# ShijieZhou-UCLA/feature-3dgs

Measured on NVIDIA H100. Metric: views/sec fwd+bwd @1M Gaussians/1080p/feat_dim=128, higher is better.
Workload: dtype f32

## Files before the change

### feature-3dgs_b200/csrc/composite_common.cuh

```cuda
#pragma once
#include <initializer_list>

#include "kernels.h"

namespace f3dgs {

constexpr int kBlocksPerTile = 8;
constexpr int kProducerWarp = 0;
constexpr int kAlphaWarp0 = 4;
constexpr int kAlphaWarps = kBlocksPerTile;
constexpr int kFeatWarp0 = kAlphaWarp0 + kAlphaWarps;
constexpr int kRegsProducer = 40;
constexpr int kStageEntries = 32;
constexpr int kStages = 6;
constexpr int kWSlots = 2;
constexpr int kDoneSlots = 8;

template <int CH, typename TF = float>
struct alignas(128) Stage {
    TF feat[CH > 0 ? kStageEntries : 1][CH > 0 ? CH : 4];
    float4 rec0[kStageEntries];
    float4 rec1[kStageEntries];
    float4 rec2[kStageEntries];
    uint32_t listpos[kStageEntries];
    uint32_t gid[kStageEntries];
    uint32_t n;
    uint32_t last;
    uint32_t first;
    int32_t work;
    uint32_t done_slot;
};

struct alignas(128) WSlot {
    float w[kStageEntries][32];
    uint32_t pm[kStageEntries];
    uint32_t km[2];
    uint32_t last;
    uint32_t first;
    int32_t work;
};
static_assert(sizeof(WSlot) == 4352, "weight slot layout changed");

constexpr int kPrefetch = 4;
struct alignas(16) RecQueue {
    float4 q[kPrefetch][3][32];
    uint32_t id[kPrefetch][32];
};

template <int CH, typename TF = float, int WB = kBlocksPerTile, int WJ = kWSlots>
struct alignas(128) RingV2 {
    using Feat = TF;
    static constexpr int kWB = WB, kWJ = WJ;
    Stage<CH, TF> stage[kStages];
    WSlot ws[WB][WJ];
    uint64_t full[kStages];
    uint64_t empty[kStages];
    uint64_t listed[kStages];
    uint64_t wfull[WB][WJ];
    uint64_t wempty[WB][WJ];
    uint32_t done_mask[kDoneSlots];
    RecQueue rq;
};

using RingSlim = RingV2<0, float, 1, 1>;

static_assert(sizeof(RecQueue) == 6656, "record queue layout changed");
static_assert(sizeof(RingV2<0>) == 88320 && sizeof(RingSlim) == 22784, "ring layout changed");
static_assert(sizeof(RingV2<32>) == 112896 && sizeof(RingV2<64>) == 137472 && sizeof(RingV2<128>) == 186624,
              "ring layout changed");
static_assert(sizeof(RingV2<32, __half>) == 100608 && sizeof(RingV2<64, __half>) == 112896 &&
                  sizeof(RingV2<128, __half>) == 137472,
              "ring layout changed");

__device__ __forceinline__ int block_x0(int tile_x, int b) { return tile_x * 16 + (b & 1) * 8; }
__device__ __forceinline__ int block_y0(int tile_y, int b) { return tile_y * 16 + (b >> 1) * 4; }
__device__ __forceinline__ int slot_px(int p) { return ((p >> 2) & 3) * 2 + (p & 1); }
__device__ __forceinline__ int slot_py(int p) { return (p >> 4) * 2 + ((p >> 1) & 1); }

template <int NQ>
__device__ __forceinline__ float& tile_px(float2 (&t)[NQ][2][4], int qi, int i, int c) {
    return (i & 1) ? t[qi][i >> 1][c].y : t[qi][i >> 1][c].x;
}
template <int NQ>
__device__ __forceinline__ float& tile_run_px(float2 (&t)[NQ][2][4], int y, int half, int k, int c) {
    return tile_px(t, ((y >> 1) * 4 + half * 2 + (k >> 1)) % NQ, (y & 1) * 2 + (k & 1), c);
}
template <int NQ>
__device__ __forceinline__ float4 tile_run(float2 (&t)[NQ][2][4], int y, int half, int c) {
    return make_float4(tile_run_px(t, y, half, 0, c), tile_run_px(t, y, half, 1, c), tile_run_px(t, y, half, 2, c),
                       tile_run_px(t, y, half, 3, c));
}
template <int NQ>
__device__ __forceinline__ void set_tile_run(float2 (&t)[NQ][2][4], int y, int half, int c, float4 v) {
    tile_run_px(t, y, half, 0, c) = v.x;
    tile_run_px(t, y, half, 1, c) = v.y;
    tile_run_px(t, y, half, 2, c) = v.z;
    tile_run_px(t, y, half, 3, c) = v.w;
}

template <int G, int NQ, int NY = 4, typename T, class Row, class Run, class Px>
__device__ __forceinline__ void for_tile_pixels(T* plane, int bx0, int by0, int W, int H, int grp, bool rows, bool runs,
                                                Row row, Run run, Px px) {
    static_assert(NQ * G * 2 == NY * 4, "a register tile of NQ quads per lane group covers NY rows of 8 pixels");
    if (G == 1 && rows && bx0 + 8 <= W) {
#pragma unroll
        for (int y = 0; y < NY; y++) {
            const int yy = by0 + y;
            if (yy >= H) continue;
            row(plane + (size_t)yy * W + bx0, y);
        }
    } else if (G == 1 && runs) {
#pragma unroll
        for (int y = 0; y < NY; y++) {
            const int yy = by0 + y;
            if (yy >= H) continue;
#pragma unroll
            for (int half = 0; half < 2; half++) {
                const int xx = bx0 + half * 4;
                if (xx >= W) continue;
                run(plane + (size_t)yy * W + xx, y, half);
            }
        }
    } else {
#pragma unroll
        for (int qi = 0; qi < NQ; qi++) {
            const int q = qi * G + grp;
#pragma unroll
            for (int i = 0; i < 4; i++) {
                const int xx = bx0 + (q & 3) * 2 + (i & 1), yy = by0 + (q >> 2) * 2 + (i >> 1);
                if (xx < W && yy < H) px(plane + (size_t)yy * W + xx, qi, i);
            }
        }
    }
}

__device__ __forceinline__ float4 to_float4(float4 v) { return v; }
__device__ __forceinline__ float4 to_float4(uint2 v) {
    const float2 a = __half22float2(*reinterpret_cast<const __half2*>(&v.x));
    const float2 b = __half22float2(*reinterpret_cast<const __half2*>(&v.y));
    return make_float4(a.x, a.y, b.x, b.y);
}

struct InstanceLists {
    float* w;
    uint2* meta;
    uint32_t* cnt;
};

__device__ __forceinline__ size_t list_begin(uint32_t begin, uint32_t end, int b) {
    return kBlocksPerTile * (size_t)begin + (size_t)b * (end - begin);
}

struct ListLayout {
    size_t w, meta, cnt, bytes;
    ListLayout(size_t R, size_t tiles) {
        size_t o = 0;
        w = o;     o = align_up(o + kBlocksPerTile * R * 32 * sizeof(float));
        meta = o;  o = align_up(o + kBlocksPerTile * R * sizeof(uint2));
        cnt = o;   o = align_up(o + kBlocksPerTile * tiles * sizeof(uint32_t));
        bytes = o;
    }
};

constexpr int kCounterFwd = 0, kCounterBwdGeom = 16, kCounterFeatureBwd = 48;

template <typename TG>
cudaError_t launch_feature_bwd(const ViewParams& vp, const uint2* ranges, const InstanceLists& lists,
                               const TG* dL_dfeat_pix, float dL_dfeat_pix_scale, float* dL_dfeature, int* counters,
                               cudaStream_t s);

struct SplatAlpha {
    float dx, dy, G, alpha;
};
__device__ __forceinline__ SplatAlpha splat_alpha(const float4 r0, const float4 r1, float pxf, float pyf, bool valid) {
    SplatAlpha s;
    s.dx = r0.x - pxf;
    s.dy = r0.y - pyf;
    const float power = -0.5f * (r1.x * s.dx * s.dx + r1.z * s.dy * s.dy) - r1.y * s.dx * s.dy;
    s.G = expf(power);
    const float av = fminf(0.99f, r1.w * s.G);
    s.alpha = (valid && !(power > 0.0f) && !(av < 1.0f / 255.0f)) ? av : 0.f;
    return s;
}

__device__ __forceinline__ bool footprint_hits_rect(const float4 r0, const float4 r1, float x0, float x1, float y0,
                                                    float y1) {
    const bool box = (r0.x + r0.z >= x0) && (r0.x - r0.z <= x1) && (r0.y + r0.w >= y0) && (r0.y - r0.w <= y1);
    if (!box) return false;
    const float dxl = r0.x - x1, dxh = r0.x - x0, dyl = r0.y - y1, dyh = r0.y - y0;
    if (r0.z > 1.0e30f || (dxl <= 0.f && dxh >= 0.f && dyl <= 0.f && dyh >= 0.f)) return true;
    const float a = r1.x, b = r1.y, c = r1.z;
    const float tau = 2.02f * __logf(255.0f * r1.w) + 0.02f;
    const float nb_ia = -b * rcp_approx(a), nb_ic = -b * rcp_approx(c);
    float q = 3.0e38f;
#pragma unroll
    for (int k = 0; k < 2; k++) {
        const float ex_ = k ? dxh : dxl;
        const float ty = fminf(fmaxf(nb_ic * ex_, dyl), dyh);
        q = fminf(q, a * ex_ * ex_ + (2.f * b * ex_ + c * ty) * ty);
        const float ey_ = k ? dyh : dyl;
        const float tx = fminf(fmaxf(nb_ia * ey_, dxl), dxh);
        q = fminf(q, c * ey_ * ey_ + (2.f * b * ey_ + a * tx) * tx);
    }
    return q <= tau;
}

enum RoleClock {
    kClkProdEmpty, kClkProdLoop,
    kClkAlphaFull, kClkAlphaWempty, kClkAlphaLoop,
    kClkFeatWfull, kClkFeatFull, kClkFeatLoop,
    kRoleClocks
};
#ifdef F3DGS_ROLE_CLOCKS
static __device__ unsigned long long g_role_clocks[kRoleClocks];
#define ROLE_CLK(...) __VA_ARGS__
#define ROLE_CLK_WAIT(acc, wait)                      \
    do {                                              \
        const uint32_t clk_t_ = (uint32_t)clock64();  \
        wait;                                         \
        acc += (uint32_t)clock64() - clk_t_;          \
    } while (0)
#define ROLE_CLK_ADD(slot, cycles) atomicAdd(&g_role_clocks[slot], (unsigned long long)(cycles))
#define ROLE_CLK_EXPORT(name)                                                                              \
    extern "C" int name(unsigned long long* out, int reset) {                                              \
        cudaError_t e = cudaMemcpyFromSymbol(out, f3dgs::g_role_clocks, sizeof(f3dgs::g_role_clocks));     \
        const unsigned long long zero[f3dgs::kRoleClocks] = {};                                            \
        if (e == cudaSuccess && reset) e = cudaMemcpyToSymbol(f3dgs::g_role_clocks, zero, sizeof(zero));   \
        return (int)e;                                                                                     \
    }
#else
#define ROLE_CLK(...)
#define ROLE_CLK_WAIT(acc, wait) wait
#endif

__device__ __forceinline__ void cp_async16(void* dst_smem, const void* src_gmem) {
    asm volatile("cp.async.ca.shared.global [%0], [%1], 16;" ::"r"(smem_u32(dst_smem)), "l"(src_gmem) : "memory");
}
__device__ __forceinline__ void cp_async_commit() { asm volatile("cp.async.commit_group;" ::: "memory"); }
template <int N>
__device__ __forceinline__ void cp_async_wait() {
    asm volatile("cp.async.wait_group %0;" ::"n"(N) : "memory");
}
__device__ __forceinline__ void cp_async_wait_pending(uint32_t n) {
    static_assert(kPrefetch <= 4, "one case per count below kPrefetch - 1");
    if (n >= (uint32_t)kPrefetch - 1u) cp_async_wait<kPrefetch - 1>();
    else if (n == 2) cp_async_wait<2>();
    else if (n == 1) cp_async_wait<1>();
    else cp_async_wait<0>();
}

template <int N>
__device__ __forceinline__ void reg_dec() {
    asm volatile("setmaxnreg.dec.sync.aligned.u32 %0;" ::"n"(N));
}
template <int N>
__device__ __forceinline__ void reg_inc() {
    asm volatile("setmaxnreg.inc.sync.aligned.u32 %0;" ::"n"(N));
}

template <int CH, typename RING>
__device__ __forceinline__ void ring_init(RING& ring, int n_stage_consumers, int n_full_arrivals = 1,
                                          int n_wslot_consumers = 1) {
    if (threadIdx.x == 0) {
        for (int s = 0; s < kStages; s++) {
            mbar_init(&ring.full[s], n_full_arrivals);
            mbar_init(&ring.empty[s], n_stage_consumers);
            mbar_init(&ring.listed[s], 1);
        }
        for (int b = 0; b < RING::kWB; b++)
            for (int j = 0; j < RING::kWJ; j++) {
                mbar_init(&ring.wfull[b][j], 1);
                mbar_init(&ring.wempty[b][j], n_wslot_consumers);
            }
        for (int i = 0; i < kDoneSlots; i++) ring.done_mask[i] = 0;
        mbar_fence_init();
    }
    if (CH > 0) {
        float4* p = reinterpret_cast<float4*>(&ring.stage[0]);
        const int n16 = (int)(sizeof(ring.stage) / 16);
        for (int i = threadIdx.x; i < n16; i += blockDim.x) p[i] = make_float4(0.f, 0.f, 0.f, 0.f);
        asm volatile("fence.proxy.async.shared::cta;" ::: "memory");
    }
}

struct ProducerArgs {
    const uint2* ranges;
    const uint32_t* point_list;
    const SplatRec* rec;
    const void* features;
    const uint32_t* n_contrib;
    int* work_counter;
    int W, H, C;
    int tiles_x, num_tiles, chunks;
    int use_bulk;
};

inline ProducerArgs producer_args(const ViewParams& vp, const uint2* ranges, const uint32_t* point_list,
                                  const SplatRec* rec, const uint32_t* n_contrib, int* work_counter) {
    return ProducerArgs{ranges, point_list, rec, nullptr, n_contrib, work_counter, vp.W, vp.H, 0, (int)vp.grid_x,
                        (int)(vp.grid_x * vp.grid_y), 1, 0};
}

inline int channel_chunk(int C) { return C <= 32 ? 32 : (C <= 64 ? 64 : 128); }

template <auto... K>
cudaError_t device_sms(int& sms, size_t smem, int threads = 0, int min_ctas = 0) {
    static std::atomic<int> sms_of_device[64];
    int dev = 0;
    cudaGetDevice(&dev);
    if (dev < 0 || dev >= 64) return cudaErrorInvalidDevice;
    if (sms_of_device[dev].load() == 0) {
        for (const void* k : std::initializer_list<const void*>{reinterpret_cast<const void*>(K)...}) {
            const cudaError_t e = cudaFuncSetAttribute(k, cudaFuncAttributeMaxDynamicSharedMemorySize, (int)smem);
            if (e != cudaSuccess) return e;
            int ctas = min_ctas;
            if (min_ctas > 0) {
                const cudaError_t eo = cudaOccupancyMaxActiveBlocksPerMultiprocessor(&ctas, k, threads, smem);
                if (eo != cudaSuccess) return eo;
            }
            if (ctas < min_ctas) return cudaErrorLaunchOutOfResources;
        }
        int n = 0;
        cudaDeviceGetAttribute(&n, cudaDevAttrMultiProcessorCount, dev);
        sms_of_device[dev].store(n > 0 ? n : 132);
    }
    sms = sms_of_device[dev].load();
    return cudaSuccess;
}

template <int CH, bool REVERSE, typename RING = RingV2<CH>>
__device__ __forceinline__ void producer_loop(RING& ring, const ProducerArgs& pa) {
    using TF = typename RING::Feat;
    constexpr bool COPYWARP = CH > 0;
    const int lane = threadIdx.x & 31;
    int s = 0;
    uint32_t empty_parity = 1;
    ROLE_CLK(uint32_t clk_empty = 0; const uint32_t clk_0 = (uint32_t)clock64();)
    ROLE_CLK_WAIT(clk_empty, mbar_wait(&ring.empty[0], empty_parity));

    uint32_t seq = 0;
    auto publish = [&](uint32_t n, uint32_t last, uint32_t first, int work) {
        __syncwarp();
        if (lane == 0) {
            Stage<CH, TF>& st = ring.stage[s];
            st.done_slot = seq % kDoneSlots;
            st.n = n;
            st.last = last;
            st.first = first;
            st.work = work;
            mbar_arrive(&ring.full[s]);
            if (COPYWARP) mbar_arrive(&ring.listed[s]);
        }
        __syncwarp();
    };
    auto advance = [&]() {
        s++;
        if (s == kStages) {
            s = 0;
            empty_parity ^= 1;
        }
        ROLE_CLK_WAIT(clk_empty, mbar_wait_sleep(&ring.empty[s], empty_parity, 64));
    };

    const int num_work = pa.num_tiles * pa.chunks;
    struct Walk {
        int work;
        uint32_t begin, count;
    };
    auto load_walk = [&](int work) {
        Walk w{work, 0u, 0u};
        if (work < num_work) {
            const int tile = work / pa.chunks;
            const uint2 range = pa.ranges[tile];
            w.begin = range.x;
            w.count = range.y - range.x;
            if (REVERSE) {
                const int tile_x = tile % pa.tiles_x, tile_y = tile / pa.tiles_x;
                uint32_t tmax = 0;
                const int yy = tile_y * 16 + (lane >> 1), xb = tile_x * 16 + (lane & 1) * 8;
                if (yy < pa.H)
                    for (int i = 0; i < 8; i++)
                        if (xb + i < pa.W) tmax = max(tmax, pa.n_contrib[(size_t)yy * pa.W + xb + i]);
#pragma unroll
                for (int o = 16; o > 0; o >>= 1) tmax = max(tmax, __shfl_xor_sync(0xffffffffu, tmax, o));
                w.count = min(w.count, tmax);
            }
        }
        return w;
    };
    auto list_index = [&](uint32_t begin, uint32_t count, uint32_t i) -> uint32_t {
        return REVERSE ? (begin + count - 1 - i) : (begin + i);
    };

    int pending = 0;
    Walk cur, nxt;
    {
        int w0 = 0, w1 = 0;
        if (lane == 0) {
            w0 = atomicAdd(pa.work_counter, 1);
            w1 = atomicAdd(pa.work_counter, 1);
            pending = atomicAdd(pa.work_counter, 1);
        }
        cur = load_walk(__shfl_sync(0xffffffffu, w0, 0));
        nxt = load_walk(__shfl_sync(0xffffffffu, w1, 0));
    }
    RecQueue& rq = ring.rq;
    uint32_t issued = 0, taken = 0;
    uint32_t ibegin = cur.begin, icount = cur.count, ic = 0, id_iss = 0;
    bool in_nxt = false;
    auto load_id = [&]() -> uint32_t {
        const uint32_t i = ic * 32 + lane;
        return i < icount ? pa.point_list[list_index(ibegin, icount, i)] : 0u;
    };
    auto cursor_cross = [&]() -> bool {
        if (in_nxt || ic * 32 < icount) return false;
        in_nxt = true;
        ibegin = nxt.begin;
        icount = nxt.count;
        ic = 0;
        return true;
    };
    auto issue = [&]() {
        cp_async_wait<kPrefetch - 1>();
        const uint32_t slot = issued % kPrefetch;
        if (ic * 32 + lane < icount) {
            const float4* r = reinterpret_cast<const float4*>(pa.rec + id_iss);
            cp_async16(&rq.q[slot][0][lane], r);
            cp_async16(&rq.q[slot][1][lane], r + 1);
            cp_async16(&rq.q[slot][2][lane], r + 2);
            rq.id[slot][lane] = id_iss;
        }
        cp_async_commit();
        issued++;
        ic++;
        cursor_cross();
        id_iss = load_id();
    };
    cursor_cross();
    id_iss = load_id();

    for (;;) {
        const int work = cur.work;
        if (work >= num_work) {
            publish(0, 1, 1, -1);
            break;
        }
        const int tile = work / pa.chunks, chunk = work - tile * pa.chunks;
        const int tile_x = tile % pa.tiles_x, tile_y = tile / pa.tiles_x;
        const uint32_t range_begin = cur.begin, walk_count = cur.count;
        const float tx0 = (float)(tile_x * 16), ty0 = (float)(tile_y * 16), tx1 = tx0 + 15.f, ty1 = ty0 + 15.f;
        const int chunk_off = chunk * CH;
        const int row_floats = (CH > 0 && pa.features != nullptr) ? min(CH, pa.C - chunk_off) : 0;
        seq++;
        uint32_t* done = &ring.done_mask[seq % kDoneSlots];
        if (lane == 0) *reinterpret_cast<volatile uint32_t*>(done) = 0;
        __syncwarp();

        auto store_entry = [&](uint32_t slot, uint32_t gid, uint32_t lpos, float4 r0, float4 r1, float4 r2) {
            Stage<CH, TF>& st = ring.stage[s];
            st.rec0[slot] = r0;
            st.rec1[slot] = r1;
            st.rec2[slot] = r2;
            st.listpos[slot] = lpos;
            st.gid[slot] = gid;
            if (CH > 0 && row_floats > 0) {
                const TF* src = static_cast<const TF*>(pa.features) + (size_t)gid * pa.C + chunk_off;
                if (!pa.use_bulk)
                    for (int c = 0; c < row_floats; c++) st.feat[slot][c] = __ldg(src + c);
            }
        };

        uint32_t fill = 0, first = 1;
        const uint32_t nchunks = (walk_count + 31) / 32;
        for (uint32_t c = 0; c < nchunks; c++) {
            if (*reinterpret_cast<volatile uint32_t*>(done) == (1u << kBlocksPerTile) - 1u) {
                taken += (in_nxt ? nchunks : ic) - c;
                if (!in_nxt) {
                    ic = nchunks;
                    cursor_cross();
                    id_iss = load_id();
                }
                break;
            }
            while (issued - taken < (uint32_t)kPrefetch && ic * 32 < icount) issue();
            cp_async_wait_pending(issued - taken - 1);
            __syncwarp();
            const uint32_t qs = taken % kPrefetch;
            taken++;
            const float4 a0 = rq.q[qs][0][lane], a1 = rq.q[qs][1][lane], a2 = rq.q[qs][2][lane];
            const uint32_t id_cur = rq.id[qs][lane];

            const uint32_t i0 = c * 32 + lane;
            const bool valid = i0 < walk_count;
            const bool keep = valid && footprint_hits_rect(a0, a1, tx0, tx1, ty0, ty1);
            const uint32_t m = __ballot_sync(0xffffffffu, keep);
            const uint32_t cnt = __popc(m);
            const uint32_t rank = __popc(m & ((1u << lane) - 1u));
            const uint32_t lpos = list_index(range_begin, walk_count, i0) - range_begin + 1;
            const uint32_t room = kStageEntries - fill;
            if (keep && rank < room) store_entry(fill + rank, id_cur, lpos, a0, a1, a2);
            if (cnt >= room) {
                publish(kStageEntries, 0, first, work);
                first = 0;
                advance();
                if (keep && rank >= room) store_entry(rank - room, id_cur, lpos, a0, a1, a2);
                fill = cnt - room;
            } else {
                fill += cnt;
            }
        }
        publish(fill, 1, first, work);
        advance();

        const int new_work = __shfl_sync(0xffffffffu, pending, 0);
        if (lane == 0 && new_work < num_work) pending = atomicAdd(pa.work_counter, 1);
        cur = nxt;
        nxt = load_walk(new_work);
        in_nxt = false;
        if (cursor_cross()) id_iss = load_id();
    }
    cp_async_wait<0>();
    ROLE_CLK(if (lane == 0) {
        ROLE_CLK_ADD(kClkProdEmpty, clk_empty);
        ROLE_CLK_ADD(kClkProdLoop, (uint32_t)clock64() - clk_0);
    })
}

template <int CH, typename TF>
__device__ __forceinline__ void copy_loop(RingV2<CH, TF>& ring, const ProducerArgs& pa) {
    const int lane = threadIdx.x & 31;
    int s = 0;
    uint32_t parity = 0;
    for (;;) {
        mbar_wait(&ring.listed[s], parity);
        Stage<CH, TF>& st = ring.stage[s];
        const uint32_t n = st.n;
        const int work = st.work;
        if (work < 0) {
            if (lane == 0) mbar_arrive(&ring.full[s]);
            break;
        }
        const int chunk_off = (work % pa.chunks) * CH;
        const uint32_t row_bytes = (uint32_t)min(CH, pa.C - chunk_off) * (uint32_t)sizeof(TF);
        if (pa.use_bulk && n > 0) {
            if (lane == 0) mbar_arrive_expect_tx(&ring.full[s], n * row_bytes);
            __syncwarp();
            if (lane < n)
                bulk_g2s(&st.feat[lane][0],
                         static_cast<const TF*>(pa.features) + (size_t)st.gid[lane] * pa.C + chunk_off, row_bytes,
                         &ring.full[s]);
        } else {
            if (lane == 0) mbar_arrive(&ring.full[s]);
        }
        if (++s == kStages) {
            s = 0;
            parity ^= 1;
        }
    }
}

}
```

### feature-3dgs_b200/csrc/composite_fwd.cu

```cuda
#include <type_traits>

#include "composite_common.cuh"

namespace f3dgs {

template <int CH>
constexpr int kFwdThreads = (kFeatWarp0 + (CH > 0 ? 2 : 1) * kBlocksPerTile) * 32;
template <int CH>
constexpr int kRegsAlpha = CH > 0 ? 56 : 64;
constexpr int kRegsFeature = 88;

template <typename TF>
struct FwdArgs {
    ProducerArgs pa;
    const float* bg;
    float* final_T;
    uint32_t* n_contrib;
    float* out_color;
    TF* out_feature;
    float* out_depth;
    int vec_store;
};

template <typename TF>
using Feat4 = std::conditional_t<std::is_same_v<TF, float>, float4, uint2>;
__device__ __forceinline__ uint32_t pack_half2(float a, float b) {
    const __half2 h = __floats2half2_rn(a, b);
    return *reinterpret_cast<const uint32_t*>(&h);
}
__device__ __forceinline__ void st_row(float* p, float4 a, float4 b) { st_na_f8(p, a, b); }
__device__ __forceinline__ void st_row(__half* p, float4 a, float4 b) {
    st_na_b128(p, make_uint4(pack_half2(a.x, a.y), pack_half2(a.z, a.w), pack_half2(b.x, b.y), pack_half2(b.z, b.w)));
}
__device__ __forceinline__ void st_run(float* p, float4 v) { st_na_f4(p, v); }
__device__ __forceinline__ void st_run(__half* p, float4 v) {
    st_na_b64(p, make_uint2(pack_half2(v.x, v.y), pack_half2(v.z, v.w)));
}
__device__ __forceinline__ void st_px(float* p, float v) { *p = v; }
__device__ __forceinline__ void st_px(__half* p, float v) { *p = __float2half_rn(v); }

template <int CH, typename TF>
__global__ void __launch_bounds__(kFwdThreads<CH>, 1)
composite_fwd_kernel(const FwdArgs<TF> args) {
    extern __shared__ __align__(128) unsigned char smem_raw[];
    using RING = RingV2<CH, TF>;
    RING& ring = *reinterpret_cast<RING*>(smem_raw);
    const int warp = __shfl_sync(0xffffffffu, threadIdx.x >> 5, 0);
    const int lane = threadIdx.x & 31;
    const int W = args.pa.W, H = args.pa.H, C = args.pa.C;
    const size_t HW = (size_t)H * W;

    ring_init<CH>(ring, CH > 0 ? kAlphaWarps + 2 * kBlocksPerTile : kAlphaWarps, CH > 0 ? 2 : 1, CH > 0 ? 2 : 1);
    __syncthreads();

    if (warp < kAlphaWarp0) {
        reg_dec<kRegsProducer>();
        if (warp == kProducerWarp) {
            producer_loop<CH, false>(ring, args.pa);
        } else if constexpr (CH > 0) {
            if (warp == kProducerWarp + 1) copy_loop<CH, TF>(ring, args.pa);
        }
        return;
    }

    if (warp < kFeatWarp0) {
        reg_dec<kRegsAlpha<CH>>();
        const int b = warp - kAlphaWarp0;
        int s = 0, j = 0;
        uint32_t parity = 0, wparity = 1;
        float T = 1.f, Cr = 0.f, Cg = 0.f, Cb = 0.f, Dp = 0.f, pxf = 0.f, pyf = 0.f, fbx0 = 0.f, fby0 = 0.f;
        uint32_t last_contrib = 0;
        int px = 0, py = 0, chunk = 0;
        bool done = true, inside = false, blk_done = true;
        ROLE_CLK(uint32_t clk_full = 0, clk_wempty = 0; const uint32_t clk_0 = (uint32_t)clock64();)
        for (;;) {
            ROLE_CLK_WAIT(clk_full, mbar_wait(&ring.full[s], parity));
            Stage<CH, TF>& st = ring.stage[s];
            const uint32_t n = st.n, last = st.last, first = st.first;
            const int work = st.work;
            if (work < 0) break;
            if (first) {
                const int tile = work / args.pa.chunks;
                chunk = work - tile * args.pa.chunks;
                const int tile_x = tile % args.pa.tiles_x, tile_y = tile / args.pa.tiles_x;
                const int bx0 = block_x0(tile_x, b), by0 = block_y0(tile_y, b);
                px = bx0 + slot_px(lane);
                py = by0 + slot_py(lane);
                inside = px < W && py < H;
                pxf = (float)px; pyf = (float)py;
                fbx0 = (float)bx0; fby0 = (float)by0;
                T = 1.f; Cr = Cg = Cb = Dp = 0.f;
                last_contrib = 0;
                done = !inside;
                blk_done = __all_sync(0xffffffffu, done);
                if (blk_done && lane == 0) atomicOr(&ring.done_mask[st.done_slot], 1u << b);
            }
            WSlot* ws = &ring.ws[b][j];
            if (CH > 0) ROLE_CLK_WAIT(clk_wempty, mbar_wait(&ring.wempty[b][j], wparity));
            uint32_t km0 = 0, km1 = 0;
            if (!blk_done && n > 0) {
                bool hit = false;
                if (lane < n) hit = footprint_hits_rect(st.rec0[lane], st.rec1[lane], fbx0, fbx0 + 7.f, fby0, fby0 + 3.f);
                uint32_t am = __ballot_sync(0xffffffffu, hit);
                while (am) {
                    int kk[4];
                    bool vk[4];
                    float al[4];
#pragma unroll
                    for (int u = 0; u < 4; u++) {
                        vk[u] = am != 0;
                        kk[u] = vk[u] ? (__ffs(am) - 1) : 0;
                        am &= am - 1;
                    }
#pragma unroll
                    for (int u = 0; u < 4; u++) al[u] = splat_alpha(st.rec0[kk[u]], st.rec1[kk[u]], pxf, pyf, vk[u]).alpha;
#pragma unroll
                    for (int u = 0; u < 4; u++) {
                        if (!vk[u]) break;
                        const float4 r2 = st.rec2[kk[u]];
                        const uint32_t lp = st.listpos[kk[u]];
                        const float alpha = al[u];
                        const float test_T = T * (1 - alpha);
                        const bool act = !done && alpha > 0.f;
                        const bool stop = act && (test_T < 0.0001f);
                        const bool blend = act && !stop;
                        done = done || stop;
                        const float wgt = blend ? alpha * T : 0.f;
                        const float nCr = Cr + r2.x * alpha * T;
                        const float nCg = Cg + r2.y * alpha * T;
                        const float nCb = Cb + r2.z * alpha * T;
                        const float nDp = Dp + r2.w * (alpha * T);
                        Cr = blend ? nCr : Cr;
                        Cg = blend ? nCg : Cg;
                        Cb = blend ? nCb : Cb;
                        Dp = blend ? nDp : Dp;
                        T = blend ? test_T : T;
                        last_contrib = blend ? lp : last_contrib;
                        const uint32_t pm = __ballot_sync(0xffffffffu, blend);
                        if (CH > 0) {
                            ws->w[kk[u]][lane] = wgt;
                            if (lane == 0) ws->pm[kk[u]] = pm;
                            km0 |= ((pm & 0xFFFFu) ? 1u : 0u) << kk[u];
                            km1 |= ((pm >> 16) ? 1u : 0u) << kk[u];
                        }
                    }
                }
                if (__all_sync(0xffffffffu, done)) {
                    blk_done = true;
                    if (lane == 0) atomicOr(&ring.done_mask[st.done_slot], 1u << b);
                }
            }
            if (CH > 0) {
                __syncwarp();
                if (lane == 0) {
                    ws->km[0] = km0;
                    ws->km[1] = km1;
                    ws->last = last;
                    ws->first = first;
                    ws->work = work;
                    mbar_arrive(&ring.wfull[b][j]);
                }
            }
            __syncwarp();
            if (lane == 0) mbar_arrive(&ring.empty[s]);
            if (last && chunk == 0 && inside) {
                const size_t pix = (size_t)py * W + px;
                args.final_T[pix] = T;
                args.n_contrib[pix] = last_contrib;
                args.out_color[pix] = Cr + T * args.bg[0];
                args.out_color[HW + pix] = Cg + T * args.bg[1];
                args.out_color[2 * HW + pix] = Cb + T * args.bg[2];
                args.out_depth[pix] = Dp;
            }
            if (++s == kStages) { s = 0; parity ^= 1; }
            if (CH > 0 && ++j == kWSlots) { j = 0; wparity ^= 1; }
        }
        ROLE_CLK(if (lane == 0) {
            ROLE_CLK_ADD(kClkAlphaFull, clk_full);
            ROLE_CLK_ADD(kClkAlphaWempty, clk_wempty);
            ROLE_CLK_ADD(kClkAlphaLoop, (uint32_t)clock64() - clk_0);
        })
        if (CH > 0) {
            mbar_wait(&ring.wempty[b][j], wparity);
            if (lane == 0) {
                ring.ws[b][j].work = -1;
                ring.ws[b][j].km[0] = ring.ws[b][j].km[1] = 0;
                mbar_arrive(&ring.wfull[b][j]);
            }
        }
        return;
    }

    if (CH == 0) return;
    reg_inc<kRegsFeature>();
    {
        constexpr int LPR = CH > 0 ? CH / 4 : 32;
        constexpr int G = 32 / LPR;
        constexpr int NQ = 4 / G;
        const int b = (warp - kFeatWarp0) >> 1, h = (warp - kFeatWarp0) & 1;
        const int grp = lane / LPR, cl = lane % LPR;
        float2 acc2[NQ][2][4];
#pragma unroll
        for (int q = 0; q < NQ; q++)
#pragma unroll
            for (int i = 0; i < 4; i++)
#pragma unroll
                for (int c = 0; c < 4; c++) tile_px(acc2, q, i, c) = 0.f;
#define FEAT_ROW_FMA(Q, ROW, W2)                                                                     \
        do {                                                                                             \
            const float2 w2_ = (W2);                                                                     \
            const float fr_[4] = {f.x, f.y, f.z, f.w};                                                   \
            _Pragma("unroll") for (int c_ = 0; c_ < 4; c_++)                                             \
                acc2[Q][ROW][c_] = fma2_rn(make_float2(fr_[c_], fr_[c_]), w2_, acc2[Q][ROW][c_]);     \
        } while (0)
        int s = 0, j = 0;
        uint32_t parity = 0, wparity = 0;
        ROLE_CLK(uint32_t clk_wfull = 0, clk_full = 0; const uint32_t clk_0 = (uint32_t)clock64();)
        for (;;) {
            ROLE_CLK_WAIT(clk_wfull, mbar_wait(&ring.wfull[b][j], wparity));
            const WSlot& ws = ring.ws[b][j];
            const int work = ws.work;
            if (work < 0) break;
            uint32_t km = ws.km[h];
            const uint32_t last = ws.last;
            ROLE_CLK_WAIT(clk_full, mbar_wait(&ring.full[s], parity));
            const Stage<CH, TF>& st = ring.stage[s];
            int kn = km ? __ffs(km) - 1 : 0;
            uint32_t pm_n = ws.pm[kn];
            Feat4<TF> f_n = *reinterpret_cast<const Feat4<TF>*>(&st.feat[kn][cl * 4]);
            while (km) {
                const int k = kn;
                const uint32_t pm = pm_n >> (16 * h);
                const float4 f = to_float4(f_n);
                km &= km - 1;
                kn = km ? __ffs(km) - 1 : k;
                pm_n = ws.pm[kn];
                f_n = *reinterpret_cast<const Feat4<TF>*>(&st.feat[kn][cl * 4]);
#pragma unroll
                for (int qi = 0; qi < NQ; qi++) {
                    const int q = qi * G + grp;
                    if ((pm >> (4 * q)) & 0xFu) {
                        const float4 w4 = *reinterpret_cast<const float4*>(&ws.w[k][16 * h + 4 * q]);
                        if ((pm >> (4 * q)) & 0x3u) FEAT_ROW_FMA(qi, 0, make_float2(w4.x, w4.y));
                        if ((pm >> (4 * q)) & 0xCu) FEAT_ROW_FMA(qi, 1, make_float2(w4.z, w4.w));
                    }
                }
            }
            __syncwarp();
            if (lane == 0) {
                mbar_arrive(&ring.wempty[b][j]);
                mbar_arrive(&ring.empty[s]);
            }
            if (last) {
                const int tile = work / args.pa.chunks, chunk = work - tile * args.pa.chunks;
                const int tile_x = tile % args.pa.tiles_x, tile_y = tile / args.pa.tiles_x;
                const int bx0 = block_x0(tile_x, b), by0 = block_y0(tile_y, b) + 2 * h;
#pragma unroll
                for (int c = 0; c < 4; c++) {
                    const int ch = chunk * CH + cl * 4 + c;
                    if (ch < C)
                        for_tile_pixels<G, NQ, 2>(
                            args.out_feature + (size_t)ch * HW, bx0, by0, W, H, grp, args.vec_store & 2,
                            args.vec_store & 1,
                            [&](TF* p, int y) { st_row(p, tile_run(acc2, y, 0, c), tile_run(acc2, y, 1, c)); },
                            [&](TF* p, int y, int half) { st_run(p, tile_run(acc2, y, half, c)); },
                            [&](TF* p, int qi, int i) { st_px(p, tile_px(acc2, qi, i, c)); });
                }
#pragma unroll
                for (int q = 0; q < NQ; q++)
#pragma unroll
                    for (int i = 0; i < 4; i++)
#pragma unroll
                        for (int c = 0; c < 4; c++) tile_px(acc2, q, i, c) = 0.f;
            }
            if (++s == kStages) { s = 0; parity ^= 1; }
            if (++j == kWSlots) { j = 0; wparity ^= 1; }
        }
        ROLE_CLK(if (lane == 0) {
            ROLE_CLK_ADD(kClkFeatWfull, clk_wfull);
            ROLE_CLK_ADD(kClkFeatFull, clk_full);
            ROLE_CLK_ADD(kClkFeatLoop, (uint32_t)clock64() - clk_0);
        })
    }
#undef FEAT_ROW_FMA
}

template <int CH, typename TF>
static cudaError_t launch_fwd_t(const ViewParams& vp, const uint2* ranges, const uint32_t* point_list,
                                const SplatRec* rec, const TF* features, const float* bg, float* final_T,
                                uint32_t* n_contrib, float* out_color, TF* out_feature, float* out_depth,
                                int* work_counter, cudaStream_t s) {
    const size_t smem = sizeof(RingV2<CH, TF>);
    int num_sms = 0;
    cudaError_t e = device_sms<composite_fwd_kernel<CH, TF>>(num_sms, smem);
    if (e != cudaSuccess) return e;
    FwdArgs<TF> a;
    a.pa = producer_args(vp, ranges, point_list, rec, nullptr, work_counter);
    a.pa.features = CH > 0 ? features : nullptr;
    a.pa.C = vp.C;
    a.pa.chunks = CH > 0 ? (vp.C + CH - 1) / CH : 1;
    constexpr int kPer16 = 16 / (int)sizeof(TF);
    a.pa.use_bulk = (CH > 0 && vp.C % kPer16 == 0 && (reinterpret_cast<uintptr_t>(features) & 15) == 0) ? 1 : 0;
    a.bg = bg; a.final_T = final_T; a.n_contrib = n_contrib;
    a.out_color = out_color; a.out_feature = out_feature; a.out_depth = out_depth;
    const uintptr_t out_addr = reinterpret_cast<uintptr_t>(out_feature);
    a.vec_store = (vp.W % 4 == 0 && (out_addr & (4 * sizeof(TF) - 1)) == 0) ? 1 : 0;
    if (vp.W % 8 == 0 && (out_addr & (8 * sizeof(TF) - 1)) == 0) a.vec_store |= 2;
    e = cudaMemsetAsync(work_counter, 0, sizeof(int), s);
    if (e != cudaSuccess) return e;
    const int grid = min(a.pa.num_tiles * a.pa.chunks, num_sms);
    composite_fwd_kernel<CH, TF><<<grid, kFwdThreads<CH>, smem, s>>>(a);
    g_launches++;
    return cudaGetLastError();
}

template <typename TF>
cudaError_t launch_composite_fwd(const ViewParams& vp, const uint2* ranges, const uint32_t* point_list,
                                 const SplatRec* rec, const TF* features, const float* bg,
                                 float* final_T, uint32_t* n_contrib, float* out_color,
                                 TF* out_feature, float* out_depth, int* counters, cudaStream_t s) {
    int* const work_counter = counters + kCounterFwd;
    if (vp.C == 0)
        return launch_fwd_t<0, float>(vp, ranges, point_list, rec, nullptr, bg, final_T, n_contrib, out_color, nullptr,
                                      out_depth, work_counter, s);
    const int ch = channel_chunk(vp.C);
    const auto launch = ch == 32 ? launch_fwd_t<32, TF> : ch == 64 ? launch_fwd_t<64, TF> : launch_fwd_t<128, TF>;
    return launch(vp, ranges, point_list, rec, features, bg, final_T, n_contrib, out_color, out_feature, out_depth,
                  work_counter, s);
}

template cudaError_t launch_composite_fwd<float>(const ViewParams&, const uint2*, const uint32_t*, const SplatRec*,
                                                 const float*, const float*, float*, uint32_t*, float*, float*, float*,
                                                 int*, cudaStream_t);
template cudaError_t launch_composite_fwd<__half>(const ViewParams&, const uint2*, const uint32_t*, const SplatRec*,
                                                  const __half*, const float*, float*, uint32_t*, float*, __half*,
                                                  float*, int*, cudaStream_t);

}

#ifdef F3DGS_ROLE_CLOCKS
ROLE_CLK_EXPORT(f3dgs_role_clocks_fwd)
#endif
```

Baseline: 154.7.

## Split feature-row barrier from stage-full barrier and deepen weight-slot ring

```diff
diff --git a/feature-3dgs_b200/csrc/composite_common.cuh b/feature-3dgs_b200/csrc/composite_common.cuh
--- a/feature-3dgs_b200/csrc/composite_common.cuh
+++ b/feature-3dgs_b200/csrc/composite_common.cuh
@@ -13,7 +13,8 @@
 constexpr int kRegsProducer = 40;
 constexpr int kStageEntries = 32;
 constexpr int kStages = 6;
-constexpr int kWSlots = 2;
+template <int CH>
+constexpr int kWSlots = CH > 0 ? 3 : 2;
 constexpr int kDoneSlots = 8;
 
 template <int CH, typename TF = float>
@@ -47,7 +48,7 @@
     uint32_t id[kPrefetch][32];
 };
 
-template <int CH, typename TF = float, int WB = kBlocksPerTile, int WJ = kWSlots>
+template <int CH, typename TF = float, int WB = kBlocksPerTile, int WJ = kWSlots<CH>>
 struct alignas(128) RingV2 {
     using Feat = TF;
     static constexpr int kWB = WB, kWJ = WJ;
@@ -60,17 +61,19 @@
     uint64_t wempty[WB][WJ];
     uint32_t done_mask[kDoneSlots];
     RecQueue rq;
+    uint64_t rows[kStages];
 };
 
 using RingSlim = RingV2<0, float, 1, 1>;
 
 static_assert(sizeof(RecQueue) == 6656, "record queue layout changed");
 static_assert(sizeof(RingV2<0>) == 88320 && sizeof(RingSlim) == 22784, "ring layout changed");
-static_assert(sizeof(RingV2<32>) == 112896 && sizeof(RingV2<64>) == 137472 && sizeof(RingV2<128>) == 186624,
+static_assert(sizeof(RingV2<32>) == 147840 && sizeof(RingV2<64>) == 172416 && sizeof(RingV2<128>) == 221568,
               "ring layout changed");
-static_assert(sizeof(RingV2<32, __half>) == 100608 && sizeof(RingV2<64, __half>) == 112896 &&
-                  sizeof(RingV2<128, __half>) == 137472,
+static_assert(sizeof(RingV2<32, __half>) == 135552 && sizeof(RingV2<64, __half>) == 147840 &&
+                  sizeof(RingV2<128, __half>) == 172416,
               "ring layout changed");
+static_assert(sizeof(RingV2<128>) <= 232448, "above the H100's 227 KiB of opt-in shared memory per block");
 
 __device__ __forceinline__ int block_x0(int tile_x, int b) { return tile_x * 16 + (b & 1) * 8; }
 __device__ __forceinline__ int block_y0(int tile_y, int b) { return tile_y * 16 + (b >> 1) * 4; }
@@ -208,7 +211,7 @@
 enum RoleClock {
     kClkProdEmpty, kClkProdLoop,
     kClkAlphaFull, kClkAlphaWempty, kClkAlphaLoop,
-    kClkFeatWfull, kClkFeatFull, kClkFeatLoop,
+    kClkFeatWfull, kClkFeatRows, kClkFeatLoop,
     kRoleClocks
 };
 #ifdef F3DGS_ROLE_CLOCKS
@@ -259,13 +262,13 @@
 }
 
 template <int CH, typename RING>
-__device__ __forceinline__ void ring_init(RING& ring, int n_stage_consumers, int n_full_arrivals = 1,
-                                          int n_wslot_consumers = 1) {
+__device__ __forceinline__ void ring_init(RING& ring, int n_stage_consumers, int n_wslot_consumers = 1) {
     if (threadIdx.x == 0) {
         for (int s = 0; s < kStages; s++) {
-            mbar_init(&ring.full[s], n_full_arrivals);
+            mbar_init(&ring.full[s], 1);
             mbar_init(&ring.empty[s], n_stage_consumers);
             mbar_init(&ring.listed[s], 1);
+            if (CH > 0) mbar_init(&ring.rows[s], 1);
         }
         for (int b = 0; b < RING::kWB; b++)
             for (int j = 0; j < RING::kWJ; j++) {
@@ -526,8 +529,8 @@
     })
 }
 
-template <int CH, typename TF>
-__device__ __forceinline__ void copy_loop(RingV2<CH, TF>& ring, const ProducerArgs& pa) {
+template <int CH, typename TF, int WJ>
+__device__ __forceinline__ void copy_loop(RingV2<CH, TF, kBlocksPerTile, WJ>& ring, const ProducerArgs& pa) {
     const int lane = threadIdx.x & 31;
     int s = 0;
     uint32_t parity = 0;
@@ -536,21 +539,18 @@
         Stage<CH, TF>& st = ring.stage[s];
         const uint32_t n = st.n;
         const int work = st.work;
-        if (work < 0) {
-            if (lane == 0) mbar_arrive(&ring.full[s]);
-            break;
-        }
+        if (work < 0) break;
         const int chunk_off = (work % pa.chunks) * CH;
         const uint32_t row_bytes = (uint32_t)min(CH, pa.C - chunk_off) * (uint32_t)sizeof(TF);
         if (pa.use_bulk && n > 0) {
-            if (lane == 0) mbar_arrive_expect_tx(&ring.full[s], n * row_bytes);
+            if (lane == 0) mbar_arrive_expect_tx(&ring.rows[s], n * row_bytes);
             __syncwarp();
             if (lane < n)
                 bulk_g2s(&st.feat[lane][0],
                          static_cast<const TF*>(pa.features) + (size_t)st.gid[lane] * pa.C + chunk_off, row_bytes,
-                         &ring.full[s]);
+                         &ring.rows[s]);
         } else {
-            if (lane == 0) mbar_arrive(&ring.full[s]);
+            if (lane == 0) mbar_arrive(&ring.rows[s]);
         }
         if (++s == kStages) {
             s = 0;
diff --git a/feature-3dgs_b200/csrc/composite_fwd.cu b/feature-3dgs_b200/csrc/composite_fwd.cu
--- a/feature-3dgs_b200/csrc/composite_fwd.cu
+++ b/feature-3dgs_b200/csrc/composite_fwd.cu
@@ -50,7 +50,7 @@
     const int W = args.pa.W, H = args.pa.H, C = args.pa.C;
     const size_t HW = (size_t)H * W;
 
-    ring_init<CH>(ring, CH > 0 ? kAlphaWarps + 2 * kBlocksPerTile : kAlphaWarps, CH > 0 ? 2 : 1, CH > 0 ? 2 : 1);
+    ring_init<CH>(ring, CH > 0 ? kAlphaWarps + 2 * kBlocksPerTile : kAlphaWarps, CH > 0 ? 2 : 1);
     __syncthreads();
 
     if (warp < kAlphaWarp0) {
@@ -58,7 +58,7 @@
         if (warp == kProducerWarp) {
             producer_loop<CH, false>(ring, args.pa);
         } else if constexpr (CH > 0) {
-            if (warp == kProducerWarp + 1) copy_loop<CH, TF>(ring, args.pa);
+            if (warp == kProducerWarp + 1) copy_loop(ring, args.pa);
         }
         return;
     }
@@ -173,7 +173,7 @@
                 args.out_depth[pix] = Dp;
             }
             if (++s == kStages) { s = 0; parity ^= 1; }
-            if (CH > 0 && ++j == kWSlots) { j = 0; wparity ^= 1; }
+            if (CH > 0 && ++j == RING::kWJ) { j = 0; wparity ^= 1; }
         }
         ROLE_CLK(if (lane == 0) {
             ROLE_CLK_ADD(kClkAlphaFull, clk_full);
@@ -215,7 +215,7 @@
         } while (0)
         int s = 0, j = 0;
         uint32_t parity = 0, wparity = 0;
-        ROLE_CLK(uint32_t clk_wfull = 0, clk_full = 0; const uint32_t clk_0 = (uint32_t)clock64();)
+        ROLE_CLK(uint32_t clk_wfull = 0, clk_rows = 0; const uint32_t clk_0 = (uint32_t)clock64();)
         for (;;) {
             ROLE_CLK_WAIT(clk_wfull, mbar_wait(&ring.wfull[b][j], wparity));
             const WSlot& ws = ring.ws[b][j];
@@ -223,7 +223,7 @@
             if (work < 0) break;
             uint32_t km = ws.km[h];
             const uint32_t last = ws.last;
-            ROLE_CLK_WAIT(clk_full, mbar_wait(&ring.full[s], parity));
+            ROLE_CLK_WAIT(clk_rows, mbar_wait(&ring.rows[s], parity));
             const Stage<CH, TF>& st = ring.stage[s];
             int kn = km ? __ffs(km) - 1 : 0;
             uint32_t pm_n = ws.pm[kn];
@@ -274,11 +274,11 @@
                         for (int c = 0; c < 4; c++) tile_px(acc2, q, i, c) = 0.f;
             }
             if (++s == kStages) { s = 0; parity ^= 1; }
-            if (++j == kWSlots) { j = 0; wparity ^= 1; }
+            if (++j == RING::kWJ) { j = 0; wparity ^= 1; }
         }
         ROLE_CLK(if (lane == 0) {
             ROLE_CLK_ADD(kClkFeatWfull, clk_wfull);
-            ROLE_CLK_ADD(kClkFeatFull, clk_full);
+            ROLE_CLK_ADD(kClkFeatRows, clk_rows);
             ROLE_CLK_ADD(kClkFeatLoop, (uint32_t)clock64() - clk_0);
         })
     }
```

Result: no change. 155.0, median of 6 (+0.2%).
